# caiyuanhao1998/Open-DiffusionGS

Hardware: AMD Instinct MI355X
Metric: novel-view renders/sec (DiT step + GS raster) at 256^2 (higher is better)
Workload: dtype bf16; 1 GPU; obj-256 sampling step (BASELINE.json configs[2]): DGSDenoiser.forward = DiT image_to_gaussians (width 1024, 24 blocks, L=4098, bf16 MFMA, fp32 accumulate) + 4 fp32 rasterizations of P=262146 Gaussians at 256^2 per sample; random-init weights; batch_per_gpu=1, views=4, resolution=256, gaussians=262146, parallelism=dp1

## Files before the change

### open-diffusiongs_amd/csrc/raster_forward.hip

```cpp
#include <string.h>

#include "raster_cells.h"

namespace dgs {

struct FwdParams {
    int P, D, M, W, H, V, vps, gx, gy, T;
    const float *bg, *means3D, *shs, *colors_pre, *opac, *scales, *rots, *cov_pre, *viewm, *projm, *campos, *tanfov;
    float tanfovx, tanfovy, scale_mod;
    int prefiltered, raw_act;
    int bin_mode;
    int bitonic_cap;
    int bitonic_any;
    int exact_exp;
    int debug;
    int* radii;
    float* out_color;
    float *out_depth, *out_alpha;
    GeomState g;
    ImageState im;
    BinningState bn;
};

__device__ __forceinline__ void view_tanfov(const FwdParams& p, int v, float* tx, float* ty) {
    if (p.tanfov) { *tx = p.tanfov[2 * v]; *ty = p.tanfov[2 * v + 1]; }
    else { *tx = p.tanfovx; *ty = p.tanfovy; }
}

__device__ __forceinline__ void sh_to_rgb(int deg, const float* sh, float dx, float dy, float dz, float* out, unsigned* clamp_bits) {
    const float len = sqrtf(dx * dx + dy * dy + dz * dz);
    const float x = dx / len, y = dy / len, z = dz / len;
    unsigned bits = 0;
#pragma unroll
    for (int c = 0; c < 3; ++c) {
#define SH(k) sh[3 * (k) + c]
        float r = 0.28209479177387814f * SH(0);
        if (deg > 0) {
            r = r - 0.4886025119029199f * y * SH(1) + 0.4886025119029199f * z * SH(2) - 0.4886025119029199f * x * SH(3);
            if (deg > 1) {
                const float xx = x * x, yy = y * y, zz = z * z, xy = x * y, yz = y * z, xz = x * z;
                r = r + 1.0925484305920792f * xy * SH(4) + -1.0925484305920792f * yz * SH(5) +
                    0.31539156525252005f * (2.0f * zz - xx - yy) * SH(6) + -1.0925484305920792f * xz * SH(7) +
                    0.5462742152960396f * (xx - yy) * SH(8);
                if (deg > 2) {
                    r = r + -0.5900435899266435f * y * (3.0f * xx - yy) * SH(9) + 2.890611442640554f * xy * z * SH(10) +
                        -0.4570457994644658f * y * (4.0f * zz - xx - yy) * SH(11) +
                        0.3731763325901154f * z * (2.0f * zz - 3.0f * xx - 3.0f * yy) * SH(12) +
                        -0.4570457994644658f * x * (4.0f * zz - xx - yy) * SH(13) + 1.445305721320277f * z * (xx - yy) * SH(14) +
                        -0.5900435899266435f * x * (xx - 3.0f * yy) * SH(15);
                }
            }
        }
#undef SH
        r += 0.5f;
        if (r < 0) bits |= 1u << c;
        out[c] = fmaxf(r, 0.0f);
    }
    *clamp_bits = bits;
}

__device__ __forceinline__ bool preprocess_one(const FwdParams& p, int v, int idx, int* rx0, int* ry0, int* rx1, int* ry1, uint32_t* depth_key) {
    const int s = v / p.vps;
    const size_t gi = (size_t)v * p.P + idx;
    const size_t si = (size_t)s * p.P + idx;
    p.radii[gi] = 0;
    p.g.tiles_touched[gi] = 0;
    p.g.keys[0][gi] = 0xFFFFFFFFu;
    const float* vm = p.viewm + 16 * v;
    const float* pm = p.projm + 16 * v;
    const float mx = p.means3D[3 * si], my = p.means3D[3 * si + 1], mz = p.means3D[3 * si + 2];
    const float hx = pm[0] * mx + pm[4] * my + pm[8] * mz + pm[12];
    const float hy = pm[1] * mx + pm[5] * my + pm[9] * mz + pm[13];
    const float hw = pm[3] * mx + pm[7] * my + pm[11] * mz + pm[15];
    const float pw = 1.0f / (hw + 0.0000001f);
    const float projx = hx * pw, projy = hy * pw;
    float tx = vm[0] * mx + vm[4] * my + vm[8] * mz + vm[12];
    float ty = vm[1] * mx + vm[5] * my + vm[9] * mz + vm[13];
    const float tz = vm[2] * mx + vm[6] * my + vm[10] * mz + vm[14];
    if (tz <= 0.2f) {
        if (p.prefiltered) p.im.totals[1] = DGS_ERR_PREFILTERED_CULLED;
        return false;
    }
    float tanx, tany;
    view_tanfov(p, v, &tanx, &tany);
    const float focal_y = p.H / (2.0f * tany), focal_x = p.W / (2.0f * tanx);

    float c6[6];
    if (p.cov_pre) {
#pragma unroll
        for (int k = 0; k < 6; ++k) c6[k] = p.cov_pre[6 * si + k];
    } else {
        cov3d_from_scale_rot(p.scales + 3 * si, p.rots + 4 * si, p.raw_act != 0, p.scale_mod, c6);
        if (p.debug) {
#pragma unroll
            for (int k = 0; k < 6; ++k) p.g.cov3D[6 * gi + k] = c6[k];
        }
    }
    const float limx = 1.3f * tanx, limy = 1.3f * tany;
    const float txtz = tx / tz, tytz = ty / tz;
    tx = fminf(limx, fmaxf(-limx, txtz)) * tz;
    ty = fminf(limy, fmaxf(-limy, tytz)) * tz;
    const M3 J = m3_cols(focal_x / tz, 0.0f, -(focal_x * tx) / (tz * tz), 0.0f, focal_y / tz, -(focal_y * ty) / (tz * tz), 0, 0, 0);
    const M3 Wm = m3_cols(vm[0], vm[4], vm[8], vm[1], vm[5], vm[9], vm[2], vm[6], vm[10]);
    const M3 Tm = m3_mul(Wm, J);
    const M3 Vrk = m3_cols(c6[0], c6[1], c6[2], c6[1], c6[3], c6[4], c6[2], c6[4], c6[5]);
    const M3 cov = m3_mul(m3_mul(m3_t(Tm), m3_t(Vrk)), Tm);
    const float ca = cov.c[0][0] + 0.3f, cb = cov.c[0][1], cc = cov.c[1][1] + 0.3f;
    const float det = ca * cc - cb * cb;
    if (det == 0.0f) return false;
    const float det_inv = 1.f / det;
    const float conx = cc * det_inv, cony = -cb * det_inv, conz = ca * det_inv;
    const float mid = 0.5f * (ca + cc);
    const float l1 = mid + sqrtf(fmaxf(0.1f, mid * mid - det));
    const float l2 = mid - sqrtf(fmaxf(0.1f, mid * mid - det));
    const float my_radius = ceilf(3.f * sqrtf(fmaxf(l1, l2)));
    const float px = (float)(((projx + 1.0) * p.W - 1.0) * 0.5);
    const float py = (float)(((projy + 1.0) * p.H - 1.0) * 0.5);
    const int irad = f2i_sat(my_radius);
    int x0, y0, x1, y1;
    tile_rect(px, py, irad, p.gx, p.gy, &x0, &y0, &x1, &y1);
    if ((x1 - x0) * (y1 - y0) == 0) return false;
    float rgb[3];
    unsigned cbits = 0;
    if (p.colors_pre) {
        rgb[0] = p.colors_pre[3 * si]; rgb[1] = p.colors_pre[3 * si + 1]; rgb[2] = p.colors_pre[3 * si + 2];
    } else {
        const float* cam = p.campos + 3 * v;
        sh_to_rgb(p.D, p.shs + 3 * (size_t)p.M * si, mx - cam[0], my - cam[1], mz - cam[2], rgb, &cbits);
    }
    float op = p.opac[si];
    if (p.raw_act) op = 1.0f / (1.0f + det_expf(-op));
    const float cut = (op > 0.0f) ? (__logf(1.0f / (255.0f * op)) - 0.004f) : __builtin_inff();
    p.g.depths[gi] = tz;
    p.radii[gi] = irad;
    p.g.means2D[gi] = make_float2(px, py);
    BlendRecord* rec = p.g.blend + gi;
    rec->co = make_float4(conx, cony, conz, op);
    rec->rc = make_float4(rgb[0], rgb[1], rgb[2], cut);
    *reinterpret_cast<float4*>(&rec->xy) = make_float4(px, py, tz, 0.f);
    p.g.clamped[gi] = (uint8_t)cbits;
    p.g.tiles_touched[gi] = (uint32_t)((y1 - y0) * (x1 - x0));
    p.g.keys[0][gi] = __float_as_uint(tz);
    *depth_key = __float_as_uint(tz);
    *rx0 = x0; *ry0 = y0; *rx1 = x1; *ry1 = y1;
    return true;
}

template <bool LDS_HIST>
__global__ __launch_bounds__(256) void preprocess_kernel(FwdParams p) {
    DGS_DYNAMIC_LDS(smem);
    uint32_t* lhist = reinterpret_cast<uint32_t*>(smem);
    const int v = blockIdx.y;
    const int idx = blockIdx.x * 256 + threadIdx.x;
    if (LDS_HIST) {
        for (int i = threadIdx.x; i < p.T; i += 256) lhist[i] = 0;
        __syncthreads();
    }
    if (blockIdx.x == 0) {
        uint32_t* w = p.g.range_ws + (size_t)v * range_ws_stride(p.P);
        for (int i = threadIdx.x; i <= kRangeBuckets; i += 256) w[i] = 0u;
    }
    int x0 = 0, y0 = 0, x1 = 0, y1 = 0;
    bool vis = false;
    uint32_t depth_key = 0xFFFFFFFFu;
    if (idx < p.P) vis = preprocess_one(p, v, idx, &x0, &y0, &x1, &y1, &depth_key);
    {
        __shared__ uint32_t s_rng[2][4];
        const uint32_t key = vis ? depth_key : 0xFFFFFFFFu;
        uint32_t hi = key != 0xFFFFFFFFu ? key : 0u, lo_c = key != 0xFFFFFFFFu ? ~key : 0u;
#pragma unroll
        for (int o = 32; o > 0; o >>= 1) { hi = max(hi, (uint32_t)__shfl_xor((int)hi, o)); lo_c = max(lo_c, (uint32_t)__shfl_xor((int)lo_c, o)); }
        if ((threadIdx.x & 63) == 0) { s_rng[0][threadIdx.x >> 6] = hi; s_rng[1][threadIdx.x >> 6] = lo_c; }
        __syncthreads();
        if (threadIdx.x < 2) {
            const uint32_t m = max(max(s_rng[threadIdx.x][0], s_rng[threadIdx.x][1]), max(s_rng[threadIdx.x][2], s_rng[threadIdx.x][3]));
            if (m) atomicMax(p.im.depth_range + ((size_t)threadIdx.x * p.V + v) * kRangeSlots + (blockIdx.x % kRangeSlots), m);
        }
    }
    uint32_t* gcount = p.im.tile_count + (size_t)v * p.T;
    if (vis) {
        uint32_t* const grid = LDS_HIST ? lhist : gcount;
        atomicAdd(&grid[y0 * p.gx + x0], 1u);
        if (x1 < p.gx) atomicAdd(&grid[y0 * p.gx + x1], 0xffffffffu);
        if (y1 < p.gy) {
            atomicAdd(&grid[y1 * p.gx + x0], 0xffffffffu);
            if (x1 < p.gx) atomicAdd(&grid[y1 * p.gx + x1], 1u);
        }
    }
    if (LDS_HIST) {
        __syncthreads();
        for (int i = threadIdx.x; i < p.T; i += 256) {
            const uint32_t c = lhist[i];
            if (c) atomicAdd(&gcount[i], c);
        }
    }
}

__global__ __launch_bounds__(256) void radix_hist_kernel(const uint32_t* keys, uint32_t* hist, int P, int NB, int shift) {
    __shared__ uint32_t h[256];
    const int v = blockIdx.y, b = blockIdx.x;
    h[threadIdx.x] = 0;
    __syncthreads();
    const uint32_t* k = keys + (size_t)v * P;
    const int base = b * kSortTile;
#pragma unroll 4
    for (int r = 0; r < kSortItems; ++r) {
        const int i = base + r * 256 + threadIdx.x;
        if (i < P) atomicAdd(&h[(k[i] >> shift) & 255u], 1u);
    }
    __syncthreads();
    hist[((size_t)v * NB + b) * 256 + threadIdx.x] = h[threadIdx.x];
}

__global__ __launch_bounds__(256) void radix_colscan_kernel(uint32_t* hist, uint32_t* base, int NB) {
    __shared__ uint32_t scratch[8];
    const int v = blockIdx.y, d = threadIdx.x;
    uint32_t* h = hist + (size_t)v * NB * 256;
    uint32_t run = 0;
    for (int b0 = 0; b0 < NB; b0 += 16) {
        uint32_t c[16];
#pragma unroll
        for (int u = 0; u < 16; ++u) c[u] = (b0 + u < NB) ? h[(size_t)(b0 + u) * 256 + d] : 0u;
#pragma unroll
        for (int u = 0; u < 16; ++u) {
            if (b0 + u < NB) h[(size_t)(b0 + u) * 256 + d] = run;
            run += c[u];
        }
    }
    uint32_t total;
    const uint32_t ex = block_exclusive_scan<256>(run, scratch, &total);
    base[v * 256 + d] = ex;
}

__global__ __launch_bounds__(256) void radix_scatter_kernel(const uint32_t* keys_in, const uint32_t* vals_in, uint32_t* keys_out,
                                                           uint32_t* vals_out, uint32_t* rank_of, const uint32_t* hist,
                                                           const uint32_t* base, int P, int NB, int shift) {
    __shared__ uint32_t wcount[4][256];
    __shared__ uint32_t running[256];
    const int v = blockIdx.y, b = blockIdx.x, tid = threadIdx.x;
    const int lane = tid & 63, wave = tid >> 6;
    const size_t vo = (size_t)v * P;
    running[tid] = base[v * 256 + tid] + hist[((size_t)v * NB + b) * 256 + tid];
    const unsigned long long lt_mask = (lane == 0) ? 0ull : (~0ull >> (64 - lane));
    for (int r = 0; r < kSortItems; ++r) {
#pragma unroll
        for (int w = 0; w < 4; ++w) wcount[w][tid] = 0;
        __syncthreads();
        const int i = b * kSortTile + r * 256 + tid;
        const bool valid = i < P;
        const uint32_t key = valid ? keys_in[vo + i] : 0xFFFFFFFFu;
        const uint32_t val = valid ? (vals_in ? vals_in[vo + i] : (uint32_t)i) : 0u;
        const uint32_t dig = (key >> shift) & 255u;
        unsigned long long peers = __ballot(valid);
#pragma unroll
        for (int bit = 0; bit < 8; ++bit) {
            const unsigned long long m = __ballot((dig >> bit) & 1u);
            peers &= ((dig >> bit) & 1u) ? m : ~m;
        }
        const uint32_t rank_in_wave = (uint32_t)__popcll(peers & lt_mask);
        if (valid && rank_in_wave == 0) wcount[wave][dig] = (uint32_t)__popcll(peers);
        __syncthreads();
        if (valid) {
            uint32_t pos = running[dig] + rank_in_wave;
            for (int w = 0; w < wave; ++w) pos += wcount[w][dig];
            keys_out[vo + pos] = key;
            vals_out[vo + pos] = val;
            if (rank_of) rank_of[vo + val] = pos;
        }
        __syncthreads();
        running[tid] += wcount[0][tid] + wcount[1][tid] + wcount[2][tid] + wcount[3][tid];
    }
}

struct RangeMap {
    uint32_t lo; float scale; bool any;
    __device__ __forceinline__ uint32_t bucket(uint32_t key) const { return min((uint32_t)((float)(key - lo) * scale), (uint32_t)kRangeBuckets - 1u); }
};
__device__ __forceinline__ RangeMap range_map(const uint32_t* depth_range, int V, int v, uint32_t* s_map ) {
    if (threadIdx.x < 64) {
        const int which = threadIdx.x >> 5, slot = threadIdx.x & 31;
        uint32_t x = slot < kRangeSlots ? depth_range[((size_t)which * V + v) * kRangeSlots + slot] : 0u;
#pragma unroll
        for (int o = 16; o > 0; o >>= 1) x = max(x, (uint32_t)__shfl_xor((int)x, o));
        if (slot == 0) s_map[which] = x;
    }
    __syncthreads();
    const uint32_t hi_w = s_map[0], lo_w = s_map[1];
    const uint32_t hi = hi_w, lo = ~lo_w;
    RangeMap m;
    m.any = (hi_w | lo_w) != 0u;
    m.lo = m.any ? lo : 0u;
    m.scale = m.any ? (float)kRangeBuckets / ((float)(hi - lo) + 1.0f) : 0.f;
    return m;
}

__global__ __launch_bounds__(256) void range_count_kernel(const uint32_t* keys, const uint32_t* depth_range, uint32_t* ws, int P, int V, int stride) {
    __shared__ uint32_t h[kRangeBuckets];
    __shared__ uint32_t s_c[4];
    __shared__ uint32_t s_map[2];
    const int v = blockIdx.y, b = blockIdx.x, tid = threadIdx.x;
    const RangeMap m = range_map(depth_range, V, v, s_map);
    for (int i = tid; i < kRangeBuckets; i += 256) h[i] = 0;
    __syncthreads();
    const uint32_t* k = keys + (size_t)v * P;
    uint32_t culled = 0;
#pragma unroll 4
    for (int r = 0; r < kRangeItems; ++r) {
        const int i = b * kRangeTile + r * 256 + tid;
        if (i < P) {
            const uint32_t key = k[i];
            if (key != 0xFFFFFFFFu) atomicAdd(&h[m.bucket(key)], 1u); else ++culled;
        }
    }
#pragma unroll
    for (int o = 32; o > 0; o >>= 1) culled += (uint32_t)__shfl_xor((int)culled, o);
    if ((tid & 63) == 0) s_c[tid >> 6] = culled;
    __syncthreads();
    uint32_t* w = ws + (size_t)v * stride;
    for (int i = tid; i < kRangeBuckets; i += 256) { const uint32_t c = h[i]; if (c) atomicAdd(&w[i], c); }
    if (tid == 0) w[2 * kRangeBuckets + 1 + b] = (s_c[0] + s_c[1]) + (s_c[2] + s_c[3]);
}

__global__ __launch_bounds__(1024) void range_plan_kernel(uint32_t* ws, int NB, int NWIN, int stride) {
    __shared__ uint32_t scratch[20];
    __shared__ uint32_t s_start[kRangeBuckets + 1];
    uint32_t* w = ws + (size_t)blockIdx.x * stride;
    const int tid = threadIdx.x;
    const uint32_t c = tid < kRangeBuckets ? w[tid] : 0u;
    uint32_t nvis;
    const uint32_t ex = block_exclusive_scan<1024>(c, scratch, &nvis);
    __syncthreads();
    if (tid < kRangeBuckets) { w[tid] = ex; w[kRangeBuckets + 1 + tid] = 0u; s_start[tid] = ex; }
    if (tid == 0) { w[kRangeBuckets] = nvis; s_start[kRangeBuckets] = nvis; }
    __syncthreads();
    for (int j = tid; j <= NWIN; j += 1024) {
        const uint32_t want = (uint32_t)j * (uint32_t)kRangeWindow;
        int lo = 0, hi = kRangeBuckets;
        while (lo < hi) { const int mid = (lo + hi) >> 1; if (s_start[mid] < want) lo = mid + 1; else hi = mid; }
        w[2 * kRangeBuckets + 1 + NB + j] = j == NWIN ? nvis : s_start[lo];
    }
    const uint32_t cc = tid < NB ? w[2 * kRangeBuckets + 1 + tid] : 0u;
    uint32_t all;
    const uint32_t cex = block_exclusive_scan<1024>(cc, scratch, &all);
    if (tid < NB) w[2 * kRangeBuckets + 1 + tid] = nvis + cex;
}

__global__ __launch_bounds__(256) void range_scatter_kernel(const uint32_t* keys, const uint32_t* depth_range, uint32_t* ws, uint32_t* keys_out,
                                                           uint32_t* vals_out, uint32_t* order, uint32_t* rank_of, int P, int V, int stride) {
    __shared__ uint32_t h[kRangeBuckets];
    __shared__ uint32_t s_cc[kRangeItems][4];
    __shared__ uint32_t s_map[2];
    const int v = blockIdx.y, b = blockIdx.x, tid = threadIdx.x, lane = tid & 63, wave = tid >> 6;
    const RangeMap m = range_map(depth_range, V, v, s_map);
    const size_t vo = (size_t)v * P;
    uint32_t* w = ws + (size_t)v * stride;
    for (int i = tid; i < kRangeBuckets; i += 256) h[i] = 0;
    __syncthreads();
    uint32_t key[kRangeItems], slot[kRangeItems];
    const unsigned long long lt_mask = (lane == 0) ? 0ull : (~0ull >> (64 - lane));
#pragma unroll
    for (int r = 0; r < kRangeItems; ++r) {
        const int i = b * kRangeTile + r * 256 + tid;
        key[r] = i < P ? keys[vo + i] : 0u;
        const bool in = i < P, cul = in && key[r] == 0xFFFFFFFFu;
        slot[r] = (in && !cul) ? atomicAdd(&h[m.bucket(key[r])], 1u) : 0u;
        const unsigned long long cm = __ballot(cul);
        if (cul) slot[r] = (uint32_t)__popcll(cm & lt_mask);
        if (lane == 0) s_cc[r][wave] = (uint32_t)__popcll(cm);
    }
    __syncthreads();
    {
        constexpr int Q = kRangeBuckets / 256;
        uint32_t c[Q], st0[Q], got[Q];
#pragma unroll
        for (int q = 0; q < Q; ++q) { c[q] = h[tid + 256 * q]; st0[q] = w[tid + 256 * q]; }
#pragma unroll
        for (int q = 0; q < Q; ++q) got[q] = c[q] ? atomicAdd(&w[kRangeBuckets + 1 + tid + 256 * q], c[q]) : 0u;
#pragma unroll
        for (int q = 0; q < Q; ++q) h[tid + 256 * q] = st0[q] + got[q];
    }
    __syncthreads();
    const uint32_t cbase = w[2 * kRangeBuckets + 1 + b];
#pragma unroll
    for (int r = 0; r < kRangeItems; ++r) {
        const int i = b * kRangeTile + r * 256 + tid;
        if (i >= P) continue;
        if (key[r] != 0xFFFFFFFFu) {
            const uint32_t pos = h[m.bucket(key[r])] + slot[r];
            keys_out[vo + pos] = key[r];
            vals_out[vo + pos] = (uint32_t)i;
        } else {
            uint32_t off = 0;
            for (int q = 0; q < r; ++q) off += (s_cc[q][0] + s_cc[q][1]) + (s_cc[q][2] + s_cc[q][3]);
            for (int q = 0; q < wave; ++q) off += s_cc[r][q];
            const uint32_t pos = cbase + off + slot[r];
            order[vo + pos] = (uint32_t)i;
            rank_of[vo + i] = pos;
        }
    }
}

__global__ __launch_bounds__(1024) void scan_tiles_kernel(uint32_t* count, uint2* ranges, uint32_t* cursor, int n,
                                                         int32_t* totals, long long capacity, uint32_t* order, int gx, int gy,
                                                         int32_t* stats_dev, int32_t* stats_host) {
    __shared__ uint32_t scratch[20];
    __shared__ uint32_t smax;
    __shared__ uint32_t s_class[1024];
    {
        const int T = gx * gy, V = n / T;
        for (int r = threadIdx.x; r < V * gy; r += 1024) {
            uint32_t* row = count + (size_t)(r / gy) * T + (size_t)(r % gy) * gx;
            uint32_t run = 0;
            for (int x0 = 0; x0 < gx; x0 += 16) {
                uint32_t c[16];
#pragma unroll
                for (int u = 0; u < 16; ++u) c[u] = x0 + u < gx ? row[x0 + u] : 0u;
#pragma unroll
                for (int u = 0; u < 16; ++u)
                    if (x0 + u < gx) { run += c[u]; row[x0 + u] = run; }
            }
        }
        __syncthreads();
        for (int cidx = threadIdx.x; cidx < V * gx; cidx += 1024) {
            uint32_t* col = count + (size_t)(cidx / gx) * T + (cidx % gx);
            uint32_t run = 0;
            for (int y0 = 0; y0 < gy; y0 += 16) {
                uint32_t c[16];
#pragma unroll
                for (int u = 0; u < 16; ++u) c[u] = y0 + u < gy ? col[(size_t)(y0 + u) * gx] : 0u;
#pragma unroll
                for (int u = 0; u < 16; ++u)
                    if (y0 + u < gy) { run += c[u]; col[(size_t)(y0 + u) * gx] = run; }
            }
        }
        __syncthreads();
    }
    uint32_t carry = 0, mx = 0;
    if (threadIdx.x == 0) smax = 0;
    for (int base = 0; base < n; base += 1024) {
        const int i = base + threadIdx.x;
        const uint32_t c = (i < n) ? count[i] : 0u;
        mx = max(mx, c);
        uint32_t tot;
        const uint32_t ex = block_exclusive_scan<1024>(c, scratch, &tot);
        if (i < n) { ranges[i] = make_uint2(carry + ex, carry + ex + c); cursor[i] = 0; }
        carry += tot;
    }
    __syncthreads();
    atomicMax(&smax, mx);
    __syncthreads();
    if (threadIdx.x == 0) {
        totals[0] = (int32_t)carry;
        totals[2] = (int32_t)smax;
        if (capacity >= 0 && (long long)carry > capacity) totals[1] = DGS_ERR_BINNING_OVERFLOW;
        const int32_t st1 = totals[1];
        if (stats_dev) { stats_dev[0] = (int32_t)carry; stats_dev[1] = st1; stats_dev[2] = (int32_t)smax; stats_dev[3] = 1; }
        if (stats_host) {
            stats_host[0] = (int32_t)carry; stats_host[1] = st1; stats_host[2] = (int32_t)smax;
            __threadfence_system();
            *reinterpret_cast<volatile int32_t*>(stats_host + 3) = 1;
        }
    }
    deal_tiles(count, n, smax, order, s_class, scratch);
}

enum { kFormRankSort = 1, kFormScan = 2, kFormBitonic = 3 };
__host__ __device__ __forceinline__ int binning_form_of(int bin_mode, int bitonic_cap, long long num_rendered, long long longest,
                                                        long long T, long long P, long long V, bool any_len = false) {
    const bool fits = bitonic_cap > 0 && (any_len || longest <= bitonic_cap);
    if (bin_mode == kFormScan || bin_mode == kFormRankSort) return bin_mode;
    if (bin_mode == kFormBitonic) return fits ? kFormBitonic : kFormRankSort;
    if (num_rendered * 10 >= T * P * V) return kFormScan;
    return fits ? kFormBitonic : kFormRankSort;
}
__host__ __device__ __forceinline__ bool scan_form_possible(int gx, int gy, long long T, long long P) {
    return gx <= 255 && gy <= 255 && T * P <= (1ll << 31);
}
__device__ __forceinline__ int binning_form(const FwdParams& p) {
    return binning_form_of(p.bin_mode, p.bitonic_cap, (long long)(uint32_t)p.im.totals[0], (long long)(uint32_t)p.im.totals[2], p.T, p.P, p.V,
                           p.bitonic_any != 0);
}
__device__ __forceinline__ bool binning_is_scan(const FwdParams& p) { return binning_form(p) == kFormScan; }

template <bool LDS_AGG>
__global__ __launch_bounds__(256) void emit_instances_kernel(FwdParams p) {
    DGS_DYNAMIC_LDS(smem);
    uint32_t* lcnt = reinterpret_cast<uint32_t*>(smem);
    uint32_t* lbase = lcnt + p.T;
    const int form = binning_form(p);
    if (p.im.totals[1] != 0 || form == kFormScan) return;
    const bool wide = form == kFormBitonic;
    const int v = blockIdx.y;
    const int idx = blockIdx.x * 256 + threadIdx.x;
    const size_t gi = (size_t)v * p.P + idx;
    int x0 = 0, y0 = 0, x1 = 0, y1 = 0;
    bool vis = false;
    if (idx < p.P && p.radii[gi] > 0) {
        const float2 m = p.g.means2D[gi];
// ... 421 lines not shown
            const uint32_t x0 = r[u] & 255u, y0 = (r[u] >> 8) & 255u, x1 = (r[u] >> 16) & 255u, y1 = r[u] >> 24;
            const unsigned long long m = __ballot(tx - x0 < x1 - x0) & __ballot(ty - y0 < y1 - y0);
            if (EMIT) {
                const bool set = (m >> lane) & 1ull;
                slot[u] = off + cnt + (uint32_t)__popcll(m & lanes_before);
                val[u] = set ? order[rank0 + 64u * u] : 0u;
                setm |= (uint32_t)set << u;
            }
            cnt += (uint32_t)__popcll(m);
        }
        if (EMIT) {
#pragma unroll
            for (int u = 0; u < 8; ++u)
                if (((setm >> u) & 1u) && list_at + slot[u] < list_cap) {
                    ring[(ring_at + slot[u]) & (kRing - 1u)] = val[u];
                    list[list_at + slot[u]] = val[u];
                }
        }
    }
    return cnt;
}

__device__ __forceinline__ void scan_more(const FwdParams& p, TileScan& s, uint32_t* ring, uint32_t* scratch, const uint32_t* rects,
                                          const uint32_t* order, uint32_t* list, uint32_t count, uint32_t tx, uint32_t ty, int lane, int wave,
                                          unsigned long long lanes_before) {
    const uint32_t P = (uint32_t)p.P;
    unsigned long long want = 768ull * P / (count ? count : 1u);
    uint32_t win = (uint32_t)(want > (1ull << 24) ? (1ull << 24) : want);
    win = max(1024u, (win + 255u) & ~255u);
    const uint32_t room = kRing - s.waiting;
    uint32_t total = 0, off = 0;
    int g0 = 0, g1 = 0;
    for (;;) {
        const int groups = (int)((min(win, P - s.next_rank) + 63u) / 64u);
        const int gpw = (groups + 3) / 4;
        g0 = wave * gpw; g1 = min(groups, g0 + gpw);
        const uint32_t cnt = scan_groups<false>(rects, order, s.next_rank, g0, g1, P, tx, ty, lane, lanes_before, 0u, nullptr, 0u, nullptr, 0u, 0u);
        if (lane == 0) scratch[wave] = cnt;
        __syncthreads();
        total = 0; off = 0;
#pragma unroll
        for (int w = 0; w < 4; ++w) {
            const uint32_t c = scratch[w];
            if (w < wave) off += c;
            total += c;
        }
        __syncthreads();
        if (total <= room || win <= 256u) break;
        win = max(256u, (win / 2u + 255u) & ~255u);
    }
    scan_groups<true>(rects, order, s.next_rank, g0, g1, P, tx, ty, lane, lanes_before, off, ring, s.head + s.waiting, list, s.found, count);
    __syncthreads();
    s.next_rank += min(win, P - s.next_rank);
    s.found += total;
    s.waiting += total;
}

template <bool SCAN, bool FAST_EXP, bool AUX = false>
__global__ __launch_bounds__(256) void blend_forward_kernel(FwdParams p) {
    __shared__ CellXY<AUX> s_xy[256];
    __shared__ float4 s_co[256];
    __shared__ float4 s_rgbc[256];
    __shared__ uint4 s_cnt[16];
    __shared__ uint8_t s_list[17][256];
    __shared__ uint32_t s_walk[4];
    __shared__ uint2 s_stat[kRasterStats ? 4 : 1];
    __shared__ uint32_t s_ring[SCAN ? kRing : 1];
    __shared__ uint32_t s_scan[4];
    if (binning_is_scan(p) != SCAN) return;
    const uint32_t vt = p.im.tile_order[blockIdx.x];
    const int v = (int)(vt / (uint32_t)p.T), tile = (int)(vt % (uint32_t)p.T);
    const int bx = tile % p.gx, by = tile / p.gx;
    const int tid = threadIdx.x, lane = tid & 63, row = lane >> 4;
    const int wave = __builtin_amdgcn_readfirstlane(tid >> 6);
    const int cell = wave * 4 + row;
    const int pxi = bx * kTile + 4 * row + (lane & 3), pyi = by * kTile + 4 * wave + ((lane >> 2) & 3);
    const bool inside = pxi < p.W && pyi < p.H;
    const float pfx = (float)pxi, pfy = (float)pyi;
    const float tx0 = (float)(bx * kTile), ty0 = (float)(by * kTile);
    const unsigned long long lanes_before = (lane == 0) ? 0ull : (~0ull >> (64 - lane));
    const bool ok = p.im.totals[1] == 0;
    uint2 rg = p.im.ranges[vt];
    if (!ok) rg.y = rg.x;
    const int rounds = (int)((rg.y - rg.x + 255u) / 256u);
    const size_t vo = (size_t)v * p.P;
    const uint32_t* rects = p.g.vals[1] + vo;
    const uint32_t* order = p.g.vals[0] + vo;
    TileScan ts{0u, 0u, 0u, 0u};
    bool done = !inside;
    float T = 1.0f, C0 = 0.f, C1 = 0.f, C2 = 0.f;
    float Dz = 0.f;
    uint32_t last_contributor = 0;
    uint32_t st_entries = 0, st_trips = 0, st_batches = 0;
    for (int i = 0; i < rounds; ++i) {
        if (__syncthreads_count(done) == 256) break;
        if constexpr (kRasterStats) ++st_batches;
        const uint32_t pos = rg.x + (uint32_t)i * 256u + (uint32_t)tid;
        const uint32_t need = min(256u, rg.y - rg.x - (uint32_t)i * 256u);
        if (SCAN) {
            while (ts.waiting < need && ts.next_rank < (uint32_t)p.P)
                scan_more(p, ts, s_ring, s_scan, rects, order, p.bn.point_list + rg.x, rg.y - rg.x, (uint32_t)bx, (uint32_t)by, lane, wave, lanes_before);
        }
        const bool has = pos < rg.y && (!SCAN || (uint32_t)tid < ts.waiting);
        uint32_t id = 0u;
        if (has) id = SCAN ? s_ring[(ts.head + (uint32_t)tid) & (kRing - 1u)] : p.bn.point_list[pos];
        const unsigned m16[1] = {stage_entry<AUX>(has, p.g.blend + vo, nullptr, id, tid, tx0, ty0, s_xy, s_co, s_rgbc)};
        const uint32_t kept = compact_cells<1>(m16, cell, tid, lane, wave, lanes_before, s_cnt, s_list);
        if (SCAN) { const uint32_t took = min(need, ts.waiting); ts.head += took; ts.waiting -= took; }
        const uint32_t base = (uint32_t)i * 256u;
        const unsigned long long alive = __ballot(!done);
        if (alive != 0ull) {
            const uint32_t tot = (((alive >> (16 * row)) & 0xFFFFull) != 0ull) ? kept : 0u;
            uint32_t tot_l = done ? 0u : tot;
            using Entry = CellEntry<AUX>;
            auto load = [&](uint32_t j) { return Entry{s_xy[j], s_co[j], s_rgbc[j]}; };
            auto step = [&](uint32_t k, uint32_t j, const Entry& e) {
                const float dx = e.xy.x - pfx, dy = e.xy.y - pfy;
                const float power = -0.5f * (e.co.x * dx * dx + e.co.z * dy * dy) - e.co.y * dx * dy;
                const bool pass = (k < tot_l) & !(power > 0.0f) & !(power < e.rc.w);
                if (wave_ballot(pass) != 0ull) {
                    const float alpha = alpha_clamp(e.co.w * blend_exp<FAST_EXP>(pass ? power : 0.0f, e.co.w));
                    const float test_T = T * (1 - alpha);
                    const bool contributes = pass & !(alpha < 1.0f / 255.0f);
                    const bool finishes = contributes & (test_T < 0.0001f);
                    const bool blends = contributes & !finishes;
                    tot_l = finishes ? 0u : tot_l;
                    if constexpr (FAST_EXP) {
                        const float w = blends ? alpha * T : 0.0f;
                        C0 = __builtin_fmaf(e.rc.x, w, C0); C1 = __builtin_fmaf(e.rc.y, w, C1); C2 = __builtin_fmaf(e.rc.z, w, C2);
                        if constexpr (AUX) Dz = __builtin_fmaf(e.xy.z, w, Dz);
                    } else {
                        const float c0 = C0 + e.rc.x * alpha * T, c1 = C1 + e.rc.y * alpha * T, c2 = C2 + e.rc.z * alpha * T;
                        C0 = blends ? c0 : C0;
                        C1 = blends ? c1 : C1;
                        C2 = blends ? c2 : C2;
                        if constexpr (AUX) { const float dz = Dz + e.xy.z * alpha * T; Dz = blends ? dz : Dz; }
                    }
                    T = blends ? test_T : T;
                    last_contributor = blends ? base + j + 1u : last_contributor;
                }
            };
            const uint32_t k = walk_cell(s_list[cell], load, step, [&](uint32_t at) { return wave_ballot(at < tot_l) != 0ull; });
            done = done | (tot_l != tot);
            if constexpr (kRasterStats) { st_entries += min(tot, k); st_trips += k; }
        }
    }
    if (inside) {
        const size_t pid = (size_t)p.W * pyi + pxi;
        const size_t HW = (size_t)p.H * p.W;
        p.im.final_T[(size_t)v * HW + pid] = T;
        p.im.n_contrib[(size_t)v * HW + pid] = last_contributor;
        float* out = p.out_color + (size_t)v * 3 * HW;
        const float bad = __uint_as_float(0x7FC00000u);
        out[pid] = ok ? C0 + T * p.bg[0] : bad;
        out[HW + pid] = ok ? C1 + T * p.bg[1] : bad;
        out[2 * HW + pid] = ok ? C2 + T * p.bg[2] : bad;
        if constexpr (AUX) {
            p.out_depth[(size_t)v * HW + pid] = ok ? Dz : bad;
            p.out_alpha[(size_t)v * HW + pid] = ok ? 1.0f - T : bad;
        }
    }
    uint32_t walked = last_contributor;
#pragma unroll
    for (int o = 32; o > 0; o >>= 1) walked = max(walked, (uint32_t)__shfl_xor((int)walked, o));
    uint2 stat = make_uint2(0u, 0u);
    if constexpr (kRasterStats) stat = tile_stat_sums<4>((lane & 15) == 0, st_entries, st_trips, lane, wave, s_stat);
    if (lane == 0) s_walk[wave] = walked;
    __syncthreads();
    if (tid == 0) {
        p.im.tile_work[vt] = max(max(s_walk[0], s_walk[1]), max(s_walk[2], s_walk[3]));
        p.im.tile_cursor[vt] = SCAN ? ts.found : rg.y - rg.x;
        p.im.tile_scanned[vt] = SCAN ? ts.next_rank : 0u;
        if constexpr (kRasterStats) p.im.tile_stats[vt] = make_uint4(stat.x, stat.y, SCAN ? ts.next_rank : 0u, st_batches);
    }
}

__global__ __launch_bounds__(1024) void zero_words_kernel(uint32_t* dst, int n) {
    for (int i = threadIdx.x; i < n; i += 1024) dst[i] = 0u;
}

__global__ void record_field_kernel(const BlendRecord* rec, float4* dst, size_t n, int field) {
    const size_t i = (size_t)blockIdx.x * 256 + threadIdx.x;
    if (i < n) dst[i] = field ? rec[i].rc : rec[i].co;
}

__global__ void mark_visible_kernel(int P, const float* means, const float* vm, uint8_t* present) {
    const int i = blockIdx.x * 256 + threadIdx.x;
    if (i >= P) return;
    const float mx = means[3 * i], my = means[3 * i + 1], mz = means[3 * i + 2];
    const float tz = vm[2] * mx + vm[6] * my + vm[10] * mz + vm[14];
    present[i] = !(tz <= 0.2f);
}

template <bool SCAN>
static void launch_blend_forward(const FwdParams& p, bool aux, int VT, size_t lds_pad, hipStream_t st) {
    with_flag(!p.exact_exp, [&](auto fast) {
        with_flag(aux, [&](auto ax) {
            hipLaunchKernelGGL((blend_forward_kernel<SCAN, decltype(fast)::value, decltype(ax)::value>), dim3(VT), dim3(256), lds_pad, st, p);
        });
    });
}

static int check(hipStream_t st, int debug) {
    hipError_t e = debug ? hipStreamSynchronize(st) : hipSuccess;
    if (e == hipSuccess) e = hipGetLastError();
    if (e != hipSuccess) { fprintf(stderr, "[dgs] rasterizer: HIP error %d (%s)\n", (int)e, hipGetErrorString(e)); return DGS_ERR_DEVICE; }
    return DGS_OK;
}

static int pick_window_words(int P) {
    int words = (P + 31) / 32;
    words = ((words + 255) / 256) * 256;
    const int kMax = 16128;
    return words < kMax ? words : kMax;
}

}

using namespace dgs;

extern "C" {

int dgs_abi_version(void) { return DGS_ABI_VERSION; }

const char* dgs_status_string(int s) {
    switch (s) {
        case DGS_OK: return "ok";
        case DGS_ERR_INVALID_ARGUMENT: return "invalid argument (means3D must have dimensions (num_points, 3); sizes must be positive)";
        case DGS_ERR_NEED_COLORS: return "provide exactly one of SHs or precomputed colors";
        case DGS_ERR_NEED_COVARIANCE: return "provide exactly one of scale/rotation pair or precomputed 3D covariance";
        case DGS_ERR_ALLOC: return "state-buffer allocation failed";
        case DGS_ERR_DEVICE: return "HIP device error";
        case DGS_ERR_PREFILTERED_CULLED: return "point is filtered although prefiltered is set";
        case DGS_ERR_BINNING_OVERFLOW: return "num_rendered exceeds binning capacity";
        default: return "unknown status";
    }
}

size_t dgs_raster_geom_bytes(int32_t P, int32_t V) { size_t b; GeomState::carve(nullptr, (size_t)P, (size_t)V, &b); return b; }
size_t dgs_raster_image_bytes(int32_t W, int32_t H, int32_t V) { size_t b; ImageState::carve(nullptr, (size_t)W, (size_t)H, (size_t)V, &b); return b; }
size_t dgs_raster_binning_bytes(int64_t N) { size_t b; BinningState::carve(nullptr, (size_t)(N < 1 ? 1 : N), &b); return b; }

int dgs_raster_forward(DgsRasterForwardArgs* a, dgs_stream_t stream) {
    hipStream_t st = static_cast<hipStream_t>(stream);
    if (!a || a->P < 0 || a->width <= 0 || a->height <= 0 || a->V < 1 || a->views_per_set < 1) return DGS_ERR_INVALID_ARGUMENT;
    const int P = a->P, V = a->V, W = a->width, H = a->height;
    a->num_rendered = 0;
    (void)hipGetLastError();
    if (!a->out_color || !a->geom_alloc || !a->img_alloc || !a->binning_alloc) return DGS_ERR_INVALID_ARGUMENT;
    if ((a->out_depth == nullptr) != (a->out_alpha == nullptr)) return DGS_ERR_INVALID_ARGUMENT;
    const bool aux = a->out_depth != nullptr;
    const size_t HW = (size_t)W * H;
    if (P == 0) {
        hipMemsetAsync(a->out_color, 0, (size_t)V * 3 * HW * sizeof(float), st);
        if (aux) { hipMemsetAsync(a->out_depth, 0, (size_t)V * HW * sizeof(float), st); hipMemsetAsync(a->out_alpha, 0, (size_t)V * HW * sizeof(float), st); }
        return check(st, a->debug);
    }
    if (!a->means3D || !a->opacities || !a->viewmatrix || !a->projmatrix || !a->campos || !a->background || !a->radii) return DGS_ERR_INVALID_ARGUMENT;
    if ((a->shs == nullptr) == (a->colors_precomp == nullptr)) return DGS_ERR_NEED_COLORS;
    if (a->cov3D_precomp ? (a->scales || a->rotations) : !(a->scales && a->rotations)) return DGS_ERR_NEED_COVARIANCE;
    if (a->shs && (a->M < 1 || a->D < 0 || (a->D + 1) * (a->D + 1) > a->M || a->D > 3)) return DGS_ERR_INVALID_ARGUMENT;

    FwdParams p{};
    p.P = P; p.D = a->D; p.M = a->M; p.W = W; p.H = H; p.V = V; p.vps = a->views_per_set;
    p.gx = (W + kTile - 1) / kTile; p.gy = (H + kTile - 1) / kTile; p.T = p.gx * p.gy;
    p.bg = a->background; p.means3D = a->means3D; p.shs = a->shs; p.colors_pre = a->colors_precomp; p.opac = a->opacities;
    p.scales = a->scales; p.rots = a->rotations; p.cov_pre = a->cov3D_precomp; p.viewm = a->viewmatrix; p.projm = a->projmatrix;
    p.campos = a->campos; p.tanfov = a->tanfov; p.tanfovx = a->tanfovx; p.tanfovy = a->tanfovy; p.scale_mod = a->scale_modifier;
    p.prefiltered = a->prefiltered; p.raw_act = a->raw_activations; p.radii = a->radii; p.out_color = a->out_color;
    p.out_depth = a->out_depth; p.out_alpha = a->out_alpha;
    p.exact_exp = a->exact_exp ? 1 : 0;
    p.debug = a->debug ? 1 : 0;

    size_t gbytes, ibytes;
    GeomState::carve(nullptr, (size_t)P, (size_t)V, &gbytes);
    ImageState::carve(nullptr, (size_t)W, (size_t)H, (size_t)V, &ibytes);
    void* gbuf = a->geom_alloc(gbytes, a->geom_user);
    void* ibuf = a->img_alloc(ibytes, a->img_user);
    if (!gbuf || !ibuf) return DGS_ERR_ALLOC;
    p.g = GeomState::carve(gbuf, (size_t)P, (size_t)V, nullptr);
    p.im = ImageState::carve(ibuf, (size_t)W, (size_t)H, (size_t)V, nullptr);
    const bool async = a->binning_capacity > 0;
    void* bbuf = nullptr;
    if (async) {
        bbuf = a->binning_alloc(dgs_raster_binning_bytes(a->binning_capacity), a->binning_user);
        if (!bbuf) return DGS_ERR_ALLOC;
        p.bn = BinningState::carve(bbuf, (size_t)a->binning_capacity, nullptr);
    }

    const int VT = V * p.T;
    constexpr int kBitonicMax = 16384;
    static const bool lds_ok =
        hipFuncSetAttribute(reinterpret_cast<const void*>(tile_bitonic_kernel<256>), hipFuncAttributeMaxDynamicSharedMemorySize,
                            kBitonicMax * 8 + 2 * kBuckets * 4) == hipSuccess &&
        hipFuncSetAttribute(reinterpret_cast<const void*>(tile_bitonic_kernel<1024>), hipFuncAttributeMaxDynamicSharedMemorySize,
                            kBitonicMax * 8 + 2 * kBuckets * 4) == hipSuccess &&
        hipFuncSetAttribute(reinterpret_cast<const void*>(tile_bitonic_kernel<512>), hipFuncAttributeMaxDynamicSharedMemorySize,
                            kBitonicMax * 8 + 2 * kBuckets * 4) == hipSuccess &&
        hipFuncSetAttribute(reinterpret_cast<const void*>(range_sort_kernel<512>), hipFuncAttributeMaxDynamicSharedMemorySize,
                            kRangeSortCap * 8 + 2 * kBuckets * 4) == hipSuccess;
    if (!lds_ok) { fprintf(stderr, "[dgs] rasterizer: hipFuncSetAttribute(tile_bitonic_kernel, %d bytes of LDS) failed\n", kBitonicMax * 8 + 2 * kBuckets * 4); return DGS_ERR_DEVICE; }
    hipLaunchKernelGGL(zero_words_kernel, dim3(1), dim3(1024), 0, st, p.im.tile_count, (int)p.im.zero_span((size_t)V));
    const dim3 gridP((P + 255) / 256, V);
    const bool lds_tiles = p.T <= 4096;
    if (lds_tiles) hipLaunchKernelGGL((preprocess_kernel<true>), gridP, dim3(256), (size_t)p.T * 4, st, p);
    else hipLaunchKernelGGL((preprocess_kernel<false>), gridP, dim3(256), 0, st, p);
    int rc = check(st, a->debug);
    if (rc) return rc;

    const bool can_scan = scan_form_possible(p.gx, p.gy, p.T, P);
    p.bin_mode = a->binning_form;
    if (p.bin_mode < 0 || p.bin_mode > 3 || (p.bin_mode == 0 && !can_scan) || (p.bin_mode == kFormScan && !can_scan)) p.bin_mode = can_scan ? 0 : kFormBitonic;
    int bitonic_only_cap = 0;
    if (async && p.bin_mode == kFormBitonic && a->longest_hint > 0) {
        bitonic_only_cap = 2048;
        while (bitonic_only_cap < a->longest_hint + a->longest_hint / 2 && bitonic_only_cap < kBitonicMax) bitonic_only_cap <<= 1;
    }
    hipLaunchKernelGGL(scan_tiles_kernel, dim3(1), dim3(1024), 0, st, p.im.tile_count, p.im.ranges, p.im.tile_cursor, VT, p.im.totals,
                       async ? (long long)a->binning_capacity : -1LL, p.im.tile_order, p.gx, p.gy, a->num_rendered_dev, a->num_rendered_host);
    rc = check(st, a->debug);
    if (rc) return rc;

    int forms = 0;
    static thread_local int last_form = 0;
    bool radix_done = false;
    auto radix_sort = [&]() {
        const int NB = sort_blocks(P);
        static const bool use_radix = getenv("DGS_RASTER_SORT") && !strcmp(getenv("DGS_RASTER_SORT"), "radix");
        const int RB = range_blocks(P);
        if (!use_radix && RB <= 1024) {
            const int stride = (int)range_ws_stride(P);
            hipLaunchKernelGGL(range_count_kernel, dim3(RB, V), dim3(256), 0, st, p.g.keys[0], p.im.depth_range, p.g.range_ws, P, V, stride);
            const int NWIN = range_windows(P), seg_off = 2 * kRangeBuckets + 1 + RB;
            hipLaunchKernelGGL(range_plan_kernel, dim3(V), dim3(1024), 0, st, p.g.range_ws, RB, NWIN, stride);
            hipLaunchKernelGGL(range_scatter_kernel, dim3(RB, V), dim3(256), 0, st, p.g.keys[0], p.im.depth_range, p.g.range_ws, p.g.keys[1], p.g.vals[1],
                               p.g.vals[0], p.g.rank_of, P, V, stride);
            hipLaunchKernelGGL(range_sort_kernel<512>, dim3(NWIN, V), dim3(512), kRangeSortCap * 8 + 2 * kBuckets * 4, st, p.g.range_ws, p.g.keys[1], p.g.vals[1],
                               p.g.vals[0], p.g.rank_of, P, stride, seg_off);
            radix_done = true;
            return;
        }
        for (int pass = 0; pass < 4; ++pass) {
            const int in = pass & 1, out = in ^ 1;
            hipLaunchKernelGGL(radix_hist_kernel, dim3(NB, V), dim3(256), 0, st, p.g.keys[in], p.g.radix_hist, P, NB, 8 * pass);
            hipLaunchKernelGGL(radix_colscan_kernel, dim3(1, V), dim3(256), 0, st, p.g.radix_hist, p.g.radix_base, NB);
            hipLaunchKernelGGL(radix_scatter_kernel, dim3(NB, V), dim3(256), 0, st, p.g.keys[in], pass == 0 ? (const uint32_t*)nullptr : p.g.vals[in],
                               p.g.keys[out], p.g.vals[out], pass == 3 ? p.g.rank_of : (uint32_t*)nullptr, p.g.radix_hist, p.g.radix_base, P, NB, 8 * pass);
        }
        radix_done = true;
    };
    if (!async) {
        if (last_form != kFormBitonic && p.bin_mode != kFormBitonic) radix_sort();
        int32_t tot[4] = {0, 0, 0, 0};
        if (hipMemcpyAsync(tot, p.im.totals, sizeof(tot), hipMemcpyDeviceToHost, st) != hipSuccess) return DGS_ERR_DEVICE;
        if (hipStreamSynchronize(st) != hipSuccess) return DGS_ERR_DEVICE;
        if (tot[1] != 0) return tot[1];
        a->num_rendered = (int64_t)(uint32_t)tot[0];
        a->longest_list = (int64_t)(uint32_t)tot[2];
        bbuf = a->binning_alloc(dgs_raster_binning_bytes(a->num_rendered), a->binning_user);
        if (!bbuf) return DGS_ERR_ALLOC;
        p.bn = BinningState::carve(bbuf, (size_t)(a->num_rendered < 1 ? 1 : a->num_rendered), nullptr);
        int cap = 2048;
        while (cap < tot[2] && cap < kBitonicMax) cap <<= 1;
        p.bitonic_cap = cap;
        last_form = binning_form_of(p.bin_mode, p.bitonic_cap, a->num_rendered, (uint32_t)tot[2], p.T, P, V);
        forms = 1 << last_form;
    } else {
        a->num_rendered = -1;
        a->longest_list = -1;
        p.bitonic_cap = bitonic_only_cap ? bitonic_only_cap : kBitonicMax;
        p.bitonic_any = bitonic_only_cap ? 1 : 0;
        forms = p.bin_mode ? (1 << p.bin_mode) | (p.bin_mode == kFormBitonic && !bitonic_only_cap ? 1 << kFormRankSort : 0)
                           : (1 << kFormRankSort) | (1 << kFormScan) | (1 << kFormBitonic);
    }

    size_t blend_pad = 0;
    if constexpr (kRasterAblate) { static const int pad = [] { const char* e = getenv("DGS_RASTER_FWD_LDS_PAD"); return e ? atoi(e) : 0; }(); blend_pad = (size_t)pad; }
    if ((forms & ((1 << kFormRankSort) | (1 << kFormScan))) && !radix_done) radix_sort();
    if (forms & (1 << kFormScan)) {
        hipLaunchKernelGGL(rank_rects_kernel, gridP, dim3(256), 0, st, p);
        launch_blend_forward<true>(p, aux, VT, blend_pad, st);
    }
    if (forms & ((1 << kFormRankSort) | (1 << kFormBitonic))) {
        if (lds_tiles) hipLaunchKernelGGL((emit_instances_kernel<true>), gridP, dim3(256), (size_t)p.T * 8, st, p);
        else hipLaunchKernelGGL((emit_instances_kernel<false>), gridP, dim3(256), 0, st, p);
    }
    if (forms & (1 << kFormRankSort)) {
        const int wwords = pick_window_words(P);
        hipLaunchKernelGGL(tile_sort_kernel, dim3(p.T, V), dim3(256), (size_t)wwords * 4, st, p, wwords);
    }
    if (forms & (1 << kFormBitonic)) {
        const size_t lds = (size_t)p.bitonic_cap * 8 + 2 * kBuckets * 4;
        static const int nt_env = getenv("DGS_RASTER_BITONIC_NT") ? atoi(getenv("DGS_RASTER_BITONIC_NT")) : 0;
        if (p.bitonic_cap > 8192) hipLaunchKernelGGL(tile_bitonic_kernel<1024>, dim3(VT), dim3(1024), lds, st, p);
        else if (p.bitonic_cap >= 4096 && nt_env != 256) hipLaunchKernelGGL(tile_bitonic_kernel<512>, dim3(VT), dim3(512), lds, st, p);
        else hipLaunchKernelGGL(tile_bitonic_kernel<256>, dim3(VT), dim3(256), lds, st, p);
    }
    if (forms & ((1 << kFormRankSort) | (1 << kFormBitonic))) launch_blend_forward<false>(p, aux, VT, blend_pad, st);
    return check(st, a->debug);
}

int dgs_raster_binning_form(int32_t binning_form, int64_t num_rendered, int64_t longest_list, int32_t P, int32_t W, int32_t H, int32_t V) {
    if (P < 0 || W <= 0 || H <= 0 || V < 1 || num_rendered < 0 || longest_list < 0) return DGS_ERR_INVALID_ARGUMENT;
    const int gx = (W + kTile - 1) / kTile, gy = (H + kTile - 1) / kTile;
    const long long T = (long long)gx * gy;
    const bool can_scan = scan_form_possible(gx, gy, T, P);
    int mode = binning_form;
    if (mode < 0 || mode > 3 || (mode == 0 && !can_scan) || (mode == kFormScan && !can_scan)) mode = can_scan ? 0 : kFormBitonic;
    return binning_form_of(mode, 16384, num_rendered, longest_list, T, P, V);
}

int dgs_mark_visible(int32_t P, const float* means3D, const float* viewmatrix, const float* projmatrix, uint8_t* present,
                     dgs_stream_t stream) {
    (void)projmatrix;
    if (P < 0) return DGS_ERR_INVALID_ARGUMENT;
    if (P == 0) return DGS_OK;
    if (!means3D || !viewmatrix || !present) return DGS_ERR_INVALID_ARGUMENT;
    hipStream_t st = static_cast<hipStream_t>(stream);
    hipLaunchKernelGGL(mark_visible_kernel, dim3((P + 255) / 256), dim3(256), 0, st, P, means3D, viewmatrix, present);
    return hipGetLastError() == hipSuccess ? DGS_OK : DGS_ERR_DEVICE;
}

int64_t dgs_raster_state_read(const char* name, int32_t P, int32_t W, int32_t H, int32_t V, int64_t N, const void* gbuf,
                              const void* bbuf, const void* ibuf, void* dst, int64_t dst_bytes, dgs_stream_t stream) {
    hipStream_t st = static_cast<hipStream_t>(stream);
    const GeomState g = GeomState::carve(const_cast<void*>(gbuf), (size_t)P, (size_t)V, nullptr);
    const ImageState im = ImageState::carve(const_cast<void*>(ibuf), (size_t)W, (size_t)H, (size_t)V, nullptr);
    const BinningState bn = BinningState::carve(const_cast<void*>(bbuf), (size_t)(N < 1 ? 1 : N), nullptr);
    const size_t n = (size_t)P * V, HW = (size_t)W * H * V;
    const size_t T = (size_t)((W + kTile - 1) / kTile) * ((H + kTile - 1) / kTile) * V;
    const void* src = nullptr;
    size_t bytes = 0;
    const auto is = [&](const char* s) { return strcmp(name, s) == 0; };
    if (is("depths")) { src = g.depths; bytes = n * 4; }
    else if (is("means2D")) { src = g.means2D; bytes = n * 8; }
    else if (is("conic_opacity") || is("rgb")) {
        bytes = n * 16;
        if ((int64_t)bytes > dst_bytes) return DGS_ERR_INVALID_ARGUMENT;
        if (n) hipLaunchKernelGGL(record_field_kernel, dim3((unsigned)((n + 255) / 256)), dim3(256), 0, st, g.blend, static_cast<float4*>(dst), n, is("rgb") ? 1 : 0);
        return hipGetLastError() == hipSuccess ? (int64_t)bytes : (int64_t)DGS_ERR_DEVICE;
    }
    else if (is("tiles_touched")) { src = g.tiles_touched; bytes = n * 4; }
    else if (is("clamped")) { src = g.clamped; bytes = n; }
    else if (is("cov3D")) { src = g.cov3D; bytes = n * 24; }
    else if (is("rank_of")) { src = g.rank_of; bytes = n * 4; }
    else if (is("order")) { src = g.vals[0]; bytes = n * 4; }
    else if (is("ranges")) { src = im.ranges; bytes = T * 8; }
    else if (is("n_contrib")) { src = im.n_contrib; bytes = HW * 4; }
    else if (is("final_T")) { src = im.final_T; bytes = HW * 4; }
    else if (is("list_len")) { src = im.tile_cursor; bytes = T * 4; }
    else if (is("tile_work")) { src = im.tile_work; bytes = T * 4; }
    else if (is("tile_scanned")) { src = im.tile_scanned; bytes = T * 4; }
    else if (is("tile_stats")) { src = im.tile_stats; bytes = T * 16; }
    else if (is("tile_stats_bwd")) { src = im.tile_stats + T; bytes = T * 16; }
    else if (is("point_list")) { src = bn.point_list; bytes = (size_t)(N < 0 ? 0 : N) * 4; }
    else return DGS_ERR_INVALID_ARGUMENT;
    if ((int64_t)bytes > dst_bytes) return DGS_ERR_INVALID_ARGUMENT;
    if (bytes && hipMemcpyAsync(dst, src, bytes, hipMemcpyDeviceToDevice, st) != hipSuccess) return DGS_ERR_DEVICE;
    return (int64_t)bytes;
}

}
```

Before: 725.9 renders/s.

## Load each Gaussian once per sample and preprocess all its views in one block

The preprocess kernel now launches one block row per sample instead of per view. Each thread loads means, 3D covariance, opacity and view-independent colour once and loops over that sample's views, with per-view LDS tile histograms chunked to fit in shared memory. This is meant to cut the repeated global reads and covariance math that were done once per view. In exchange the grid shrinks by the views-per-sample factor, which lowers parallelism, and LDS use grows with the view count, which may reduce occupancy.

```diff
diff --git a/open-diffusiongs_amd/csrc/raster_forward.hip b/open-diffusiongs_amd/csrc/raster_forward.hip
--- a/open-diffusiongs_amd/csrc/raster_forward.hip
+++ b/open-diffusiongs_amd/csrc/raster_forward.hip
@@ -59,16 +59,40 @@
     *clamp_bits = bits;
 }
 
-__device__ __forceinline__ bool preprocess_one(const FwdParams& p, int v, int idx, int* rx0, int* ry0, int* rx1, int* ry1, uint32_t* depth_key) {
-    const int s = v / p.vps;
-    const size_t gi = (size_t)v * p.P + idx;
-    const size_t si = (size_t)s * p.P + idx;
-    p.radii[gi] = 0;
-    p.g.tiles_touched[gi] = 0;
-    p.g.keys[0][gi] = 0xFFFFFFFFu;
+struct GaussianIn {
+    float mx, my, mz;
+    float c6[6];
+    float op, cut;
+    float rgb[3];
+    unsigned cbits;
+};
+
+__device__ __forceinline__ void load_gaussian(const FwdParams& p, size_t si, GaussianIn* g) {
+    g->mx = p.means3D[3 * si]; g->my = p.means3D[3 * si + 1]; g->mz = p.means3D[3 * si + 2];
+    if (p.cov_pre) {
+#pragma unroll
+        for (int k = 0; k < 6; ++k) g->c6[k] = p.cov_pre[6 * si + k];
+    } else {
+        cov3d_from_scale_rot(p.scales + 3 * si, p.rots + 4 * si, p.raw_act != 0, p.scale_mod, g->c6);
+    }
+    g->cbits = 0;
+    g->rgb[0] = g->rgb[1] = g->rgb[2] = 0.f;
+    if (p.colors_pre) {
+        g->rgb[0] = p.colors_pre[3 * si]; g->rgb[1] = p.colors_pre[3 * si + 1]; g->rgb[2] = p.colors_pre[3 * si + 2];
+    } else if (p.D == 0) {
+        sh_to_rgb(0, p.shs + 3 * (size_t)p.M * si, 0.f, 0.f, 1.f, g->rgb, &g->cbits);
+    }
+    float op = p.opac[si];
+    if (p.raw_act) op = 1.0f / (1.0f + det_expf(-op));
+    g->op = op;
+    g->cut = (op > 0.0f) ? (__logf(1.0f / (255.0f * op)) - 0.004f) : __builtin_inff();
+}
+
+__device__ __forceinline__ bool preprocess_view(const FwdParams& p, int v, size_t gi, size_t si, const GaussianIn& g, int* rx0, int* ry0,
+                                                int* rx1, int* ry1, uint32_t* depth_key) {
     const float* vm = p.viewm + 16 * v;
     const float* pm = p.projm + 16 * v;
-    const float mx = p.means3D[3 * si], my = p.means3D[3 * si + 1], mz = p.means3D[3 * si + 2];
+    const float mx = g.mx, my = g.my, mz = g.mz;
     const float hx = pm[0] * mx + pm[4] * my + pm[8] * mz + pm[12];
     const float hy = pm[1] * mx + pm[5] * my + pm[9] * mz + pm[13];
     const float hw = pm[3] * mx + pm[7] * my + pm[11] * mz + pm[15];
@@ -84,18 +108,11 @@
     float tanx, tany;
     view_tanfov(p, v, &tanx, &tany);
     const float focal_y = p.H / (2.0f * tany), focal_x = p.W / (2.0f * tanx);
-
-    float c6[6];
-    if (p.cov_pre) {
-#pragma unroll
-        for (int k = 0; k < 6; ++k) c6[k] = p.cov_pre[6 * si + k];
-    } else {
-        cov3d_from_scale_rot(p.scales + 3 * si, p.rots + 4 * si, p.raw_act != 0, p.scale_mod, c6);
-        if (p.debug) {
-#pragma unroll
-            for (int k = 0; k < 6; ++k) p.g.cov3D[6 * gi + k] = c6[k];
-        }
-    }
+    if (!p.cov_pre && p.debug) {
+#pragma unroll
+        for (int k = 0; k < 6; ++k) p.g.cov3D[6 * gi + k] = g.c6[k];
+    }
+    const float* c6 = g.c6;
     const float limx = 1.3f * tanx, limy = 1.3f * tany;
     const float txtz = tx / tz, tytz = ty / tz;
     tx = fminf(limx, fmaxf(-limx, txtz)) * tz;
@@ -120,23 +137,18 @@
     int x0, y0, x1, y1;
     tile_rect(px, py, irad, p.gx, p.gy, &x0, &y0, &x1, &y1);
     if ((x1 - x0) * (y1 - y0) == 0) return false;
-    float rgb[3];
-    unsigned cbits = 0;
-    if (p.colors_pre) {
-        rgb[0] = p.colors_pre[3 * si]; rgb[1] = p.colors_pre[3 * si + 1]; rgb[2] = p.colors_pre[3 * si + 2];
-    } else {
+    float rgb[3] = {g.rgb[0], g.rgb[1], g.rgb[2]};
+    unsigned cbits = g.cbits;
+    if (!p.colors_pre && p.D > 0) {
         const float* cam = p.campos + 3 * v;
         sh_to_rgb(p.D, p.shs + 3 * (size_t)p.M * si, mx - cam[0], my - cam[1], mz - cam[2], rgb, &cbits);
     }
-    float op = p.opac[si];
-    if (p.raw_act) op = 1.0f / (1.0f + det_expf(-op));
-    const float cut = (op > 0.0f) ? (__logf(1.0f / (255.0f * op)) - 0.004f) : __builtin_inff();
     p.g.depths[gi] = tz;
     p.radii[gi] = irad;
     p.g.means2D[gi] = make_float2(px, py);
     BlendRecord* rec = p.g.blend + gi;
-    rec->co = make_float4(conx, cony, conz, op);
-    rec->rc = make_float4(rgb[0], rgb[1], rgb[2], cut);
+    rec->co = make_float4(conx, cony, conz, g.op);
+    rec->rc = make_float4(rgb[0], rgb[1], rgb[2], g.cut);
     *reinterpret_cast<float4*>(&rec->xy) = make_float4(px, py, tz, 0.f);
     p.g.clamped[gi] = (uint8_t)cbits;
     p.g.tiles_touched[gi] = (uint32_t)((y1 - y0) * (x1 - x0));
@@ -146,54 +158,77 @@
     return true;
 }
 
+constexpr int kPreViews = 16;
+constexpr int kPreLdsBytes = 63 * 1024;
 template <bool LDS_HIST>
-__global__ __launch_bounds__(256) void preprocess_kernel(FwdParams p) {
+__global__ __launch_bounds__(256) void preprocess_kernel(FwdParams p, int chunk) {
     DGS_DYNAMIC_LDS(smem);
     uint32_t* lhist = reinterpret_cast<uint32_t*>(smem);
-    const int v = blockIdx.y;
-    const int idx = blockIdx.x * 256 + threadIdx.x;
-    if (LDS_HIST) {
-        for (int i = threadIdx.x; i < p.T; i += 256) lhist[i] = 0;
-        __syncthreads();
-    }
-    if (blockIdx.x == 0) {
-        uint32_t* w = p.g.range_ws + (size_t)v * range_ws_stride(p.P);
-        for (int i = threadIdx.x; i <= kRangeBuckets; i += 256) w[i] = 0u;
-    }
-    int x0 = 0, y0 = 0, x1 = 0, y1 = 0;
-    bool vis = false;
-    uint32_t depth_key = 0xFFFFFFFFu;
-    if (idx < p.P) vis = preprocess_one(p, v, idx, &x0, &y0, &x1, &y1, &depth_key);
-    {
-        __shared__ uint32_t s_rng[2][4];
-        const uint32_t key = vis ? depth_key : 0xFFFFFFFFu;
-        uint32_t hi = key != 0xFFFFFFFFu ? key : 0u, lo_c = key != 0xFFFFFFFFu ? ~key : 0u;
-#pragma unroll
-        for (int o = 32; o > 0; o >>= 1) { hi = max(hi, (uint32_t)__shfl_xor((int)hi, o)); lo_c = max(lo_c, (uint32_t)__shfl_xor((int)lo_c, o)); }
-        if ((threadIdx.x & 63) == 0) { s_rng[0][threadIdx.x >> 6] = hi; s_rng[1][threadIdx.x >> 6] = lo_c; }
-        __syncthreads();
-        if (threadIdx.x < 2) {
-            const uint32_t m = max(max(s_rng[threadIdx.x][0], s_rng[threadIdx.x][1]), max(s_rng[threadIdx.x][2], s_rng[threadIdx.x][3]));
-            if (m) atomicMax(p.im.depth_range + ((size_t)threadIdx.x * p.V + v) * kRangeSlots + (blockIdx.x % kRangeSlots), m);
-        }
-    }
-    uint32_t* gcount = p.im.tile_count + (size_t)v * p.T;
-    if (vis) {
-        uint32_t* const grid = LDS_HIST ? lhist : gcount;
-        atomicAdd(&grid[y0 * p.gx + x0], 1u);
-        if (x1 < p.gx) atomicAdd(&grid[y0 * p.gx + x1], 0xffffffffu);
-        if (y1 < p.gy) {
-            atomicAdd(&grid[y1 * p.gx + x0], 0xffffffffu);
-            if (x1 < p.gx) atomicAdd(&grid[y1 * p.gx + x1], 1u);
-        }
-    }
-    if (LDS_HIST) {
-        __syncthreads();
-        for (int i = threadIdx.x; i < p.T; i += 256) {
-            const uint32_t c = lhist[i];
-            if (c) atomicAdd(&gcount[i], c);
-        }
-    }
+    __shared__ uint32_t s_rng[kPreViews][2][4];
+    const int s = blockIdx.y, tid = threadIdx.x;
+    const int idx = blockIdx.x * 256 + tid;
+    const bool in = idx < p.P;
+    const size_t si = (size_t)s * p.P + idx;
+    GaussianIn g{};
+    if (in) load_gaussian(p, si, &g);
+    const int v_end = min((s + 1) * p.vps, p.V);
+    for (int v0 = s * p.vps; v0 < v_end; v0 += chunk) {
+        const int nv = min(chunk, v_end - v0);
+        if (LDS_HIST) {
+            for (int i = tid; i < nv * p.T; i += 256) lhist[i] = 0;
+        }
+        __syncthreads();
+        for (int j = 0; j < nv; ++j) {
+            const int v = v0 + j;
+            const size_t gi = (size_t)v * p.P + idx;
+            if (blockIdx.x == 0) {
+                uint32_t* w = p.g.range_ws + (size_t)v * range_ws_stride(p.P);
+                for (int i = tid; i <= kRangeBuckets; i += 256) w[i] = 0u;
+            }
+            int x0 = 0, y0 = 0, x1 = 0, y1 = 0;
+            uint32_t depth_key = 0xFFFFFFFFu;
+            const bool vis = in && preprocess_view(p, v, gi, si, g, &x0, &y0, &x1, &y1, &depth_key);
+            if (in && !vis) { p.radii[gi] = 0; p.g.tiles_touched[gi] = 0; p.g.keys[0][gi] = 0xFFFFFFFFu; }
+            {
+                const uint32_t key = vis ? depth_key : 0xFFFFFFFFu;
+                uint32_t hi = key != 0xFFFFFFFFu ? key : 0u, lo_c = key != 0xFFFFFFFFu ? ~key : 0u;
+#pragma unroll
+                for (int o = 32; o > 0; o >>= 1) { hi = max(hi, (uint32_t)__shfl_xor((int)hi, o)); lo_c = max(lo_c, (uint32_t)__shfl_xor((int)lo_c, o)); }
+                if ((tid & 63) == 0) { s_rng[j][0][tid >> 6] = hi; s_rng[j][1][tid >> 6] = lo_c; }
+            }
+            if (vis) {
+                uint32_t* const grid = LDS_HIST ? lhist + (size_t)j * p.T : p.im.tile_count + (size_t)v * p.T;
+                atomicAdd(&grid[y0 * p.gx + x0], 1u);
+                if (x1 < p.gx) atomicAdd(&grid[y0 * p.gx + x1], 0xffffffffu);
+                if (y1 < p.gy) {
+                    atomicAdd(&grid[y1 * p.gx + x0], 0xffffffffu);
+                    if (x1 < p.gx) atomicAdd(&grid[y1 * p.gx + x1], 1u);
+                }
+            }
+        }
+        __syncthreads();
+        if (LDS_HIST) {
+            uint32_t* gcount = p.im.tile_count + (size_t)v0 * p.T;
+            for (int i = tid; i < nv * p.T; i += 256) {
+                const uint32_t c = lhist[i];
+                if (c) atomicAdd(&gcount[i], c);
+            }
+        }
+        if (tid < 2 * nv) {
+            const int j = tid >> 1, which = tid & 1;
+            const uint32_t m = max(max(s_rng[j][which][0], s_rng[j][which][1]), max(s_rng[j][which][2], s_rng[j][which][3]));
+            if (m) atomicMax(p.im.depth_range + ((size_t)which * p.V + v0 + j) * kRangeSlots + (blockIdx.x % kRangeSlots), m);
+        }
+    }
+}
+
+static int preprocess_chunk(int vps, int T, bool lds_tiles) {
+    int chunk = vps < kPreViews ? vps : kPreViews;
+    if (lds_tiles) {
+        const int fit = kPreLdsBytes / (T * 4);
+        if (chunk > fit) chunk = fit;
+    }
+    return chunk;
 }
 
 __global__ __launch_bounds__(256) void radix_hist_kernel(const uint32_t* keys, uint32_t* hist, int P, int NB, int shift) {
@@ -1221,9 +1256,11 @@
     if (!lds_ok) { fprintf(stderr, "[dgs] rasterizer: hipFuncSetAttribute(tile_bitonic_kernel, %d bytes of LDS) failed\n", kBitonicMax * 8 + 2 * kBuckets * 4); return DGS_ERR_DEVICE; }
     hipLaunchKernelGGL(zero_words_kernel, dim3(1), dim3(1024), 0, st, p.im.tile_count, (int)p.im.zero_span((size_t)V));
     const dim3 gridP((P + 255) / 256, V);
+    const dim3 gridS((P + 255) / 256, (V + p.vps - 1) / p.vps);
     const bool lds_tiles = p.T <= 4096;
-    if (lds_tiles) hipLaunchKernelGGL((preprocess_kernel<true>), gridP, dim3(256), (size_t)p.T * 4, st, p);
-    else hipLaunchKernelGGL((preprocess_kernel<false>), gridP, dim3(256), 0, st, p);
+    const int chunk = preprocess_chunk(p.vps < V ? p.vps : V, p.T, lds_tiles);
+    if (lds_tiles) hipLaunchKernelGGL((preprocess_kernel<true>), gridS, dim3(256), (size_t)chunk * p.T * 4, st, p, chunk);
+    else hipLaunchKernelGGL((preprocess_kernel<false>), gridS, dim3(256), 0, st, p, chunk);
     int rc = check(st, a->debug);
     if (rc) return rc;
 
```

Result: no change. 728.3 renders/s (median of 6 runs) (+0.3%).
